# Mariachiar/Spatiotemporal-Deepfake-Detection-for-Live-Video-Calls

Hardware: AMD Instinct MI355X
Metric: clips/sec (32x3x224x224) (higher is better)
Workload: dtype bf16

## Files before the change

### include/af_hip.h

```cpp
#ifndef AF_HIP_H
#define AF_HIP_H

#include <stdint.h>

#ifdef __cplusplus
extern "C" {
#endif

#define AF_ABI_VERSION 6

enum af_dtype { AF_F32 = 0, AF_BF16 = 1, AF_F16 = 2 };

enum af_status {
    AF_OK = 0,
    AF_ERR_ARG = -1,
    AF_ERR_LAUNCH = -2,
    AF_ERR_NO_DEVICE = -3
};

#define AF_STEM_PAD_T 2
#define AF_STEM_PAD_H 3
#define AF_STEM_PAD_W_LEFT 3
#define AF_STEM_PAD_W_TOTAL 8
#define AF_STEM_CPAD 4
// ... 93 lines not shown

int af_conv_cpa_fusable(const af_conv_desc* dc, const af_conv_desc* da, int x_sub);
int af_conv3d_cpa_bn_act(const af_conv_desc* dc, const void* in_b, const void* wc_packed, const float* scale_c, const float* shift_c,
                         const void* residual, void* out_x, int x_sub, const af_conv_desc* da, const void* wa_packed,
                         const float* scale_a, const float* shift_a, void* out_a, void* stream);

int af_conv_variant(const af_conv_desc* d, const af_conv_desc* d2);
const char* af_conv_variant_name(int variant);

int af_maxpool3d(const af_pool_desc* d, const void* in, void* out, void* stream);

int af_avgpool_fc(const af_pool_desc* d, const void* in, const float* fc_w, const float* fc_b,
                  int num_classes, float* pooled, float* logits, void* stream);
int af_avgpool_fc_scores(const af_pool_desc* d, const void* in, const float* fc_w, const float* fc_b,
                         int num_classes, float* pooled, float* logits, float* scores, void* stream);

int af_avgpool(const af_pool_desc* d, const void* in, float* pooled, int pooled_ld, void* stream);
int af_linear(const float* x, const float* w, const float* b, int rows, int in_features, int out_features,
              float* y, void* stream);
int af_linear_scores(const float* x, const float* w, const float* b, int rows, int in_features, int out_features,
                     float* y, float* scores, void* stream);


int af_pack_tstem_weight(const float* w_oidhw, int cout, int kt, int dtype, void* out, void* stream);
long long af_packed_tstem_weight_bytes(int dtype);
int af_tstem_conv_bn_pool_relu(const af_conv_desc* d, const void* stem_in, const void* w_packed, const float* scale,
                               const float* shift, void* out, void* stream);
int af_tstem_conv_bn_pool_relu_maxpool(const af_conv_desc* d, const void* stem_in, const void* w_packed, const float* scale,
                                       const float* shift, void* out, void* stream);

// ... 105 lines not shown
    int64_t in_strides[5];
    float mean[3], std_[3];
    void* workspace;
    int64_t workspace_bytes;
    float* scores;
    const float* scale2;
    const float* shift2;
    af_conv_desc conv3;
    const void* in3;
    const void* weight3;
    const float* scale3;
    const float* shift3;
    af_conv_desc conv4;
    const void* weight4;
    int32_t x_sub;
    int32_t reserved0;
} af_op;

int af_run_ops(const af_op* ops, int n_ops, void* stream);
int af_run_ops_timed(const af_op* ops, int n_ops, void* stream, float* ms);

#define AF_YUNET_MAX_TOPK 8192
#define AF_YUNET_MAX_SIDE 8192
#define AF_YUNET_LAUNCHES 18
typedef struct af_yunet_desc {
    int32_t batch, height, width;
    int32_t top_k;
    int64_t frame_stride, row_pitch;
    float conf_threshold, nms_threshold;
} af_yunet_desc;
int64_t af_yunet_weight_floats(void);
// ... 38 lines not shown
```

### spatiotemporal-deepfake-detection-for-live-video-calls_amd/_lib.py

```python
import ctypes as C
import os

HERE = os.path.dirname(os.path.abspath(__file__))
LIB_PATH = os.environ.get("AF_HIP_LIB") or os.path.join(HERE, "libafhip.so")

AF_F32, AF_BF16, AF_F16 = 0, 1, 2
(AF_OP_STEM, AF_OP_CONV, AF_OP_MAXPOOL, AF_OP_HEAD, AF_OP_PACK_F32, AF_OP_PACK_U8, AF_OP_CONV_DUAL, AF_OP_STEM_POOL, AF_OP_AVGPOOL,
 AF_OP_LINEAR, AF_OP_TSTEM, AF_OP_TOKENS, AF_OP_LAYERNORM, AF_OP_ATTENTION, AF_OP_GELU, AF_OP_CONV_BC, AF_OP_PACK3_F32,
 AF_OP_PACK3_U8, AF_OP_STEM3_POOL, AF_OP_CONV_CA, AF_OP_BLOCK_ABC, AF_OP_TSTEM_POOL3, AF_OP_CONV_CPA) = range(23)
AF_ABI_VERSION = 6
STEM_PAD_T, STEM_PAD_H, STEM_PAD_W_LEFT, STEM_PAD_W_TOTAL, STEM_CPAD = 2, 3, 3, 8, 4

DTYPE_CODES = {"f32": AF_F32, "bf16": AF_BF16, "f16": AF_F16}


class ConvDesc(C.Structure):
    _fields_ = [(n, C.c_int32) for n in (
        "n", "t", "h", "w", "cin", "cout", "kt", "kh", "kw", "st", "sh", "sw", "pt", "ph", "pw",
        "to", "ho", "wo", "relu", "dtype", "tpool")]


class StageRect(C.Structure):
    _fields_ = [("src", C.c_void_p), ("dst_offset", C.c_int64), ("src_pitch", C.c_int64), ("rows", C.c_int32), ("row_bytes", C.c_int32)]

# ... 49 lines not shown
    _fields_ = [
        ("kind", C.c_int32), ("out_ld", C.c_int32),
        ("conv", ConvDesc), ("pool", PoolDesc),
        ("in_", C.c_void_p), ("weight", C.c_void_p), ("scale", C.c_void_p), ("shift", C.c_void_p),
        ("residual", C.c_void_p), ("out", C.c_void_p), ("aux", C.c_void_p),
        ("num_classes", C.c_int32), ("tag", C.c_int32),
        ("conv2", ConvDesc), ("in2", C.c_void_p), ("weight2", C.c_void_p),
        ("in_strides", C.c_int64 * 5),
        ("mean", C.c_float * 3), ("std_", C.c_float * 3),
        ("workspace", C.c_void_p), ("workspace_bytes", C.c_int64),
        ("scores", C.c_void_p),
        ("scale2", C.c_void_p), ("shift2", C.c_void_p),
        ("conv3", ConvDesc), ("in3", C.c_void_p), ("weight3", C.c_void_p),
        ("scale3", C.c_void_p), ("shift3", C.c_void_p),
        ("conv4", ConvDesc), ("weight4", C.c_void_p),
        ("x_sub", C.c_int32), ("reserved0", C.c_int32),
    ]


class YunetDesc(C.Structure):
    _fields_ = [("batch", C.c_int32), ("height", C.c_int32), ("width", C.c_int32), ("top_k", C.c_int32),
                ("frame_stride", C.c_int64), ("row_pitch", C.c_int64), ("conf_threshold", C.c_float), ("nms_threshold", C.c_float)]


YUNET_MAX_TOPK, YUNET_MAX_SIDE, YUNET_LAUNCHES = 8192, 8192, 18


class RetinafaceDesc(C.Structure):
    _fields_ = [("batch", C.c_int32), ("height", C.c_int32), ("width", C.c_int32), ("keep_top_k", C.c_int32),
                ("frame_stride", C.c_int64), ("row_pitch", C.c_int64), ("max_count", C.c_int32), ("reserved", C.c_int32),
                ("min_score", C.c_double)]
# ... 45 lines not shown
    "af_conv_cpa_fusable": (C.c_int, [C.POINTER(ConvDesc)] * 2 + [C.c_int]),
    "af_conv3d_cpa_bn_act": (C.c_int, [C.POINTER(ConvDesc)] + [C.c_void_p] * 6 + [C.c_int, C.POINTER(ConvDesc)] + [C.c_void_p] * 5),
    "af_conv3d_ca_bn_act": (C.c_int, [C.POINTER(ConvDesc), C.c_void_p, C.c_void_p, C.POINTER(ConvDesc)] + [C.c_void_p] * 6
                            + [C.POINTER(ConvDesc)] + [C.c_void_p] * 5),
    "af_conv_bc_fusable": (C.c_int, [C.POINTER(ConvDesc), C.POINTER(ConvDesc)]),
    "af_conv3d_bc_bn_act": (C.c_int, [C.POINTER(ConvDesc)] + [C.c_void_p] * 4 + [C.POINTER(ConvDesc)] + [C.c_void_p] * 5
                            + [C.c_int, C.c_void_p]),
    "af_block_abc_fusable": (C.c_int, [C.POINTER(ConvDesc)] * 4),
    "af_block_abc_bn_act": (C.c_int, ([C.POINTER(ConvDesc)] + [C.c_void_p] * 4) + ([C.POINTER(ConvDesc)] + [C.c_void_p] * 3) * 2
                            + [C.POINTER(ConvDesc), C.c_void_p] + [C.c_void_p, C.c_int, C.c_void_p]),
    "af_conv_variant": (C.c_int, [C.POINTER(ConvDesc), C.POINTER(ConvDesc)]),
    "af_conv_variant_name": (C.c_char_p, [C.c_int]),
    "af_maxpool3d": (C.c_int, [C.POINTER(PoolDesc), C.c_void_p, C.c_void_p, C.c_void_p]),
    "af_avgpool_fc": (C.c_int, [C.POINTER(PoolDesc)] + [C.c_void_p] * 3 + [C.c_int] + [C.c_void_p] * 3),
    "af_avgpool_fc_scores": (C.c_int, [C.POINTER(PoolDesc)] + [C.c_void_p] * 3 + [C.c_int] + [C.c_void_p] * 4),
    "af_linear_scores": (C.c_int, [C.c_void_p] * 3 + [C.c_int] * 3 + [C.c_void_p, C.c_void_p, C.c_void_p]),
    "af_masked_mean_proj": (C.c_int, [C.c_void_p, C.c_int, C.c_int, C.c_int, C.c_void_p, C.c_int, C.c_void_p, C.c_int, C.c_void_p,
                                      C.c_int, C.c_void_p]),
    "af_mlp_head": (C.c_int, [C.c_void_p, C.c_void_p, C.c_int, C.c_int, C.c_int, C.c_void_p, C.c_void_p, C.c_void_p]),
    "af_avgpool": (C.c_int, [C.POINTER(PoolDesc), C.c_void_p, C.c_void_p, C.c_int, C.c_void_p]),
    "af_linear": (C.c_int, [C.c_void_p] * 3 + [C.c_int] * 3 + [C.c_void_p, C.c_void_p]),
    "af_pack_tstem_weight": (C.c_int, [C.c_void_p, C.c_int, C.c_int, C.c_int, C.c_void_p, C.c_void_p]),
    "af_packed_tstem_weight_bytes": (C.c_longlong, [C.c_int]),
    "af_tstem_conv_bn_pool_relu": (C.c_int, [C.POINTER(ConvDesc)] + [C.c_void_p] * 6),
    "af_tstem_conv_bn_pool_relu_maxpool": (C.c_int, [C.POINTER(ConvDesc)] + [C.c_void_p] * 6),
    "af_tokens_assemble": (C.c_int, [C.c_void_p] * 3 + [C.c_int] * 3 + [C.c_void_p, C.c_void_p]),
    "af_layernorm": (C.c_int, [C.c_void_p, C.c_longlong, C.c_void_p, C.c_void_p, C.c_int, C.c_int, C.c_float, C.c_void_p,
                               C.c_longlong, C.c_void_p]),
    "af_attention": (C.c_int, [C.c_void_p, C.c_int, C.c_int, C.c_int, C.c_int, C.c_void_p, C.c_void_p]),
    "af_gelu": (C.c_int, [C.c_void_p, C.c_longlong, C.c_void_p]),
# ... 54 lines not shown
```

### spatiotemporal-deepfake-detection-for-live-video-calls_amd/csrc/af_api.hip

```cpp
#include "af_common.h"

namespace af {

static thread_local char g_err[512] = "";

int set_error(int code, const char* fmt, ...) {
    va_list ap;
    va_start(ap, fmt);
    vsnprintf(g_err, sizeof(g_err), fmt, ap);
    va_end(ap);
    return code;
}

int device_cus() {
    static int cus[kMaxDevices] = {};
    const int dev = current_device();
    if (dev >= 0 && cus[dev] > 0) return cus[dev];
    int n = 0, d = dev < 0 ? 0 : dev;
    if (dev < 0) (void)hipGetDevice(&d);
    if (hipDeviceGetAttribute(&n, hipDeviceAttributeMultiprocessorCount, d) != hipSuccess || n <= 0) n = 256;
    if (dev >= 0) cus[dev] = n;
    return n;
}

static int run_one(const af_op& op, hipStream_t s) {
    switch (op.kind) {
        case AF_OP_STEM:
            return af_stem_conv_bn_relu(&op.conv, op.in, op.weight, op.scale, op.shift, op.out, s);
        case AF_OP_STEM_POOL:
            return af_stem_conv_bn_relu_maxpool(&op.conv, op.in, op.weight, op.scale, op.shift, op.out, s);
        case AF_OP_CONV:
            return af_conv3d_bn_act(&op.conv, op.in, op.weight, op.scale, op.shift, op.residual, op.out, op.out_ld, op.workspace,
                                    op.workspace_bytes, s);
        case AF_OP_CONV_DUAL:
            return af_conv3d_dual_bn_act(&op.conv, op.in, op.weight, &op.conv2, op.in2, op.weight2, op.scale, op.shift,
                                         op.out, op.out_ld, s);
        case AF_OP_CONV_BC:
            return af_conv3d_bc_bn_act(&op.conv, op.in, op.weight, op.scale, op.shift, &op.conv2, op.weight2, op.scale2, op.shift2,
                                       op.residual, op.out, op.out_ld, s);
        case AF_OP_CONV_CPA:
            return af_conv3d_cpa_bn_act(&op.conv, op.in, op.weight, op.scale, op.shift, op.residual, op.out, op.x_sub, &op.conv2,
                                        op.weight2, op.scale2, op.shift2, op.aux, s);
        case AF_OP_CONV_CA:
            return af_conv3d_ca_bn_act(&op.conv, op.in, op.weight, op.in3 ? &op.conv3 : nullptr, op.in3, op.weight3, op.scale, op.shift,
                                       op.residual, op.out, &op.conv2, op.weight2, op.scale2, op.shift2, op.aux, s);
        case AF_OP_BLOCK_ABC:
            return af_block_abc_bn_act(&op.conv, op.in, op.weight, op.scale, op.shift, &op.conv2, op.weight2, op.scale2, op.shift2,
                                       &op.conv3, op.weight3, op.scale3, op.shift3, op.weight4 ? &op.conv4 : nullptr, op.weight4,
                                       op.out, op.out_ld, s);
        case AF_OP_MAXPOOL:
            return af_maxpool3d(&op.pool, op.in, op.out, s);
        case AF_OP_HEAD:
            return af_avgpool_fc_scores(&op.pool, op.in, (const float*)op.weight, op.scale, op.num_classes, (float*)op.aux,
                                        (float*)op.out, op.scores, s);
        case AF_OP_AVGPOOL:
            return af_avgpool(&op.pool, op.in, (float*)op.out, op.out_ld, s);
        case AF_OP_LINEAR:
            return af_linear_scores((const float*)op.in, (const float*)op.weight, op.scale, op.pool.n, op.pool.c, op.num_classes,
                                    (float*)op.out, op.scores, s);
        case AF_OP_PACK_F32:
            return af_pack_input_f32((const float*)op.in, op.conv.n, op.conv.t, op.conv.h, op.conv.w, op.in_strides[0],
                                     op.in_strides[1], op.in_strides[2], op.in_strides[3], op.in_strides[4],
                                     op.conv.dtype, op.out, s);
        case AF_OP_PACK_U8:
            return af_pack_input_u8((const uint8_t*)op.in, op.conv.n, op.conv.t, op.conv.h, op.conv.w, op.mean, op.std_,
                                    op.conv.dtype, op.out, s);
        case AF_OP_STEM3_POOL:
// ... 63 lines not shown
```

### spatiotemporal-deepfake-detection-for-live-video-calls_amd/csrc/af_conv.hip

```cpp
#include "af_common.h"

namespace af {

struct ConvArgs {
    const char* in;
    const char* w;
    const float* scale;
    const float* shift;
    const char* res;
    char* out;
    int T, H, W, Cin, Cout;
    int CinP, CoutP;
    int kt, kh, kw, st, sh, sw, pt, ph, pw;
    int To, Ho, Wo;
    int relu, out_ld;
    int ring;
    int tpool;
    long long M;
    int tiles_n;
    int kpt;
    const char* in2;
    const char* w2;
    int T2, H2, W2, Cin2, Cin2P, st2, sh2, sw2, kpt2;
    int ksplit;
    unsigned div_w_m, div_w_l, div_h_m, div_h_l, div_t_m, div_t_l;
    float* ws;
    long long ws_bytes;
#ifdef AF_STAMPS
    unsigned long long* stamps;
    int dbg;
#endif
};

template <int DT, int BN, int BM, int WN, int WM, int KS, int NSTAGE, int MINW, bool DUAL, bool SPLITK, int BMR>
__device__ __forceinline__ void conv_igemm_tile(const ConvArgs& a, const int bid, const int nb) {
    typedef Elem<DT> E;
    constexpr int EPC = E::EPC;
    constexpr int ES = 16 / EPC;
    constexpr int WTN = BN / WN, WTM = BMR / WM;
    constexpr int TN = WTN / 16, TM = WTM / 16;
    constexpr int NW = WN * WM * KS;
    constexpr int GR = NW * 8;
    constexpr int RW = BN / GR, RX = BM / GR;
    constexpr int PER_WAVE = RW + RX;
    constexpr int STAGE_BYTES = (BN + BM) * 128;
    static_assert(NW == 8 && (KS == 1 || KS == 2) && BN % GR == 0 && BM % GR == 0, "8 waves per workgroup");
    static_assert(BMR <= BM && BMR % (WM * 16) == 0, "real tile rows");
    constexpr bool LEAN = MINW >= 4;
    typedef Mma<DT> MMA;
    static_assert(NSTAGE == 3 || (NSTAGE == 2 && !LEAN && KS == 1), "ring depth of the pipelined loop: 3 or 2 slots");

    extern __shared__ uint4 smem[];
    const unsigned lds0 = (unsigned)(uintptr_t)(__attribute__((address_space(3))) char*)smem;
    AF_STAMP_DECL;
    AF_STAMP(4);

    const int xcd = bid & 7, q = nb >> 3, r = nb & 7;
    const int swz = (xcd < r ? xcd * (q + 1) : r * (q + 1) + (xcd - r) * q) + (bid >> 3);
    const int tile_n = swz % a.tiles_n;
    const int tile_m = swz / a.tiles_n;

    const int tid = threadIdx.x, lane = tid & 63;
// ... 333 lines not shown
        f32x4* red = reinterpret_cast<f32x4*>(smem);
        if (kgroup == 1) {
#pragma unroll
            for (int i = 0; i < TN; ++i)
#pragma unroll
                for (int j = 0; j < TM; ++j) red[(wsub * TN * TM + i * TM + j) * 64 + lane] = acc[i][j];
        }
        __builtin_amdgcn_s_barrier();
        if (kgroup == 1) return;
#pragma unroll
        for (int i = 0; i < TN; ++i)
#pragma unroll
            for (int j = 0; j < TM; ++j) acc[i][j] += red[(wsub * TN * TM + i * TM + j) * 64 + lane];
        patch_off = WN * WM * TN * TM * 64 * 4;
    }
    if constexpr (DT != AF_F32 && !SPLITK && KS == 1 && !LEAN) {
        if (a.tpool == 0 && !a.res) {
            typedef typename E::type OT;
            constexpr int PROW16 = WTN + 8;
            OT* patch16 = reinterpret_cast<OT*>(smem) + wsub * (16 * PROW16);
            constexpr int LPR16 = WTN / 8, RPI16 = 64 / LPR16;
            const int rr16 = lane / LPR16, cc16 = (lane % LPR16) * 8;
            const int chb = tile_n * BN + wn * WTN;
            f32x4 sc[TN], sf[TN];
#pragma unroll
            for (int i = 0; i < TN; ++i) {
                sc[i] = *reinterpret_cast<const f32x4*>(a.scale + chb + i * 16 + fg * 4);
                sf[i] = *reinterpret_cast<const f32x4*>(a.shift + chb + i * 16 + fg * 4);
            }
            const float lo = a.relu ? 0.f : -__builtin_inff();
#pragma unroll
// ... 93 lines not shown
#pragma unroll
                            for (int e = 0; e < EPC; ++e) v[p2][e] += E::to_f32(re[e]);
                        }
                    }
                    uint4 o;
                    typename E::type* oe = reinterpret_cast<typename E::type*>(&o);
#pragma unroll
                    for (int e = 0; e < EPC; ++e) {
                        float x0 = v[0][e], x1 = v[1][e];
                        if (a.relu) { x0 = relu_f(x0); x1 = relu_f(x1); }
                        oe[e] = E::from_f32(max_nan(x0, x1));
                    }
                    __builtin_nontemporal_store(__builtin_bit_cast(u32x4, o), reinterpret_cast<u32x4*>(a.out + ((m >> 1) * a.out_ld + ch0) * ES));
                }
            }
        } else {
#pragma unroll
            for (int it = 0; it < PROWS / RPI; ++it) {
                const int row = it * RPI + rr;
                const long long m = m0 + wm * WTM + hf * PROWS + row;
                float v[EPC];
#pragma unroll
                for (int e = 0; e < EPC; e += 4) {
                    const f32x4 t = *reinterpret_cast<const f32x4*>(patch + row * PROW + cc + e);
                    v[e] = t[0]; v[e + 1] = t[1]; v[e + 2] = t[2]; v[e + 3] = t[3];
                }
                if (SPLITK) {
                    if (m < a.M && ch0 < a.Cout) {
                        float* wp = a.ws + ((long long)blockIdx.y * a.M + m) * a.Cout + ch0;
#pragma unroll
// ... 13 lines not shown
                    }
                    uint4 o;
                    typename E::type* oe = reinterpret_cast<typename E::type*>(&o);
#pragma unroll
                    for (int e = 0; e < EPC; ++e) oe[e] = E::from_f32(v[e]);
                    __builtin_nontemporal_store(__builtin_bit_cast(u32x4, o), reinterpret_cast<u32x4*>(a.out + (m * a.out_ld + ch0) * ES));
                }
            }
        }
        __builtin_amdgcn_wave_barrier();
    }
    AF_STAMP(3); AF_STAMP(7);
    AF_STAMP_FLUSH(bid);
}

template <int DT, int BN, int BM, int WN, int WM, int KS, int NSTAGE, int MINW, bool DUAL, bool SPLITK, int BMR>
__global__ __launch_bounds__(WN * WM * KS * 64, MINW) void conv_igemm_kernel(const ConvArgs a) {
    conv_igemm_tile<DT, BN, BM, WN, WM, KS, NSTAGE, MINW, DUAL, SPLITK, BMR>(a, blockIdx.x, gridDim.x);
}

template <int DT, int BN, int BM, int WN, int WM, int KS, int MINW, bool DUAL, int NSTAGE = 3, bool SPLITK = false, int BMR = BM>
static int launch(const ConvArgs& a, hipStream_t stream) {
    const long long tiles_m = (a.M + BMR - 1) / BMR;
    const long long blocks = tiles_m * a.tiles_n;
    if (blocks <= 0 || blocks > 0x7fffffffLL) return set_error(AF_ERR_ARG, "conv: grid of %lld workgroups", blocks);
    constexpr int TMv = BMR / WM / 16;
    constexpr int red_bytes = KS == 2 ? WN * WM * (BN / WN / 16) * TMv * 64 * 16 : 0;
    constexpr int patch_bytes = red_bytes + WN * WM * ((TMv % 4 == 0 && TMv >= 8 ? TMv / 4 : TMv % 2 == 0 ? TMv / 2 : 1) * 16) * (BN / WN + 4) * 4;
    const int S = a.kt * a.kh * a.kw * a.kpt + a.kpt2;
    const int slots = (MINW >= 4 && a.ring == 2) ? 2 : NSTAGE;
    const int ring_bytes = (S < slots ? S : slots) * (BN + BM) * 128;
    const int lds = ring_bytes > patch_bytes ? ring_bytes : patch_bytes;
    AF_SET_MAX_LDS((&conv_igemm_kernel<DT, BN, BM, WN, WM, KS, NSTAGE, MINW, DUAL, SPLITK, BMR>),
                   NSTAGE * (BN + BM) * 128 > patch_bytes ? NSTAGE * (BN + BM) * 128 : patch_bytes, "conv");
    hipLaunchKernelGGL((conv_igemm_kernel<DT, BN, BM, WN, WM, KS, NSTAGE, MINW, DUAL, SPLITK, BMR>), dim3((unsigned)blocks, SPLITK ? a.ksplit : 1), dim3(WN * WM * KS * 64), lds, stream, a);
    AF_CHECK_LAUNCH("conv_igemm_kernel");
    return AF_OK;
}

enum { VAR_128x256 = 0, VAR_64x256 = 1, VAR_128x128 = 2, VAR_64x128 = 3, VAR_C133 = 4, VAR_128x128_R2 = 5, VAR_256x256 = 6,
       VAR_128x512 = 7, VAR_C311 = 8, VAR_SMALL = 9, VAR_C111 = 10, VAR_C133G = 11, VAR_256x224 = 12, VAR_C311G = 13, VAR_COUNT = 14 };

struct Variant { const char* name; int bn, bm, wn, wm, ks, minw, nstage, bmr, ring; bool dual; };
constexpr Variant variant_info(int v) {
    switch (v) {
        case VAR_128x256: return {"conv_igemm<BN=128,BM=256>", 128, 256, 2, 4, 1, 2, 3, 256, 3, true};
        case VAR_64x256: return {"conv_igemm<BN=64,BM=256>", 64, 256, 1, 8, 1, 2, 3, 256, 3, true};
        case VAR_128x128: return {"conv_igemm<BN=128,BM=128>", 128, 128, 2, 4, 1, 6, 3, 128, 3, true};
        case VAR_128x128_R2: return {"conv_igemm<BN=128,BM=128>", 128, 128, 2, 4, 1, 6, 3, 128, 2, true};
        case VAR_64x128: return {"conv_igemm<BN=64,BM=128>", 64, 128, 1, 8, 1, 4, 3, 128, 3, true};
// ... 91 lines not shown
    constexpr Variant t = variant_info(V < VAR_COUNT ? V : VAR_64x128);
    if constexpr (V < VAR_COUNT && (t.bn == 0 || (DUAL && !t.dual))) return launch_variant<DT, DUAL, SPLITK, V + 1>(v, a, stream);
    else {
        if constexpr (V < VAR_COUNT) if (v != V) return launch_variant<DT, DUAL, SPLITK, V + 1>(v, a, stream);
        return launch<DT, t.bn, t.bm, t.wn, t.wm, t.ks, t.minw, DUAL, t.nstage, SPLITK, t.bmr>(a, stream);
    }
}

template <int DT>
static int dispatch(ConvArgs& a, const ConvPad& p, int v, hipStream_t stream) {
    a.kpt = p.kpt; a.CinP = p.cinp; a.kpt2 = p.kpt2; a.Cin2P = p.cin2p; a.CoutP = p.coutp;
    a.tiles_n = a.CoutP / variant_bn(v);
    a.ring = variant_info(v).ring;
    a.ksplit = plan_ksplit(v, a.M, a.CoutP, a.Cout, p.ksteps, a.tpool, a.in2 != nullptr);
    if (a.ksplit > 1 && (!a.ws || a.ws_bytes < (long long)a.ksplit * a.M * a.Cout * (long long)sizeof(float))) a.ksplit = 1;
    const int rc = a.in2 ? launch_variant<DT, true, false>(v, a, stream)
                   : a.ksplit > 1 ? launch_variant<DT, false, true>(v, a, stream) : launch_variant<DT, false, false>(v, a, stream);
    if (rc != AF_OK || a.ksplit == 1) return rc;
    const long long quads = a.M * (a.Cout / 4);
    hipLaunchKernelGGL((splitk_finish_kernel<DT>), dim3((unsigned)((quads + 255) / 256)), dim3(256), 0, stream, a.ws, a.ksplit, a.M, a.Cout,
                       a.scale, a.shift, a.res, a.relu, a.out, a.out_ld);
    AF_CHECK_LAUNCH("splitk_finish_kernel");
    return AF_OK;
}

}

extern "C" int af_conv_variant(const af_conv_desc* d, const af_conv_desc* d2) {
    AF_REQUIRE(d && d->cout > 0 && d->cin > 0 && af::dtype_ok(d->dtype), "conv_variant: bad descriptor");
    return af::conv_path(d, d2, nullptr, 0, af::conv_pad(d, d2));
}

extern "C" const char* af_conv_variant_name(int variant) {
    return af::variant_info(variant).name;
}

extern "C" int64_t af_conv_workspace_bytes(const af_conv_desc* d) {
    using namespace af;
    if (!d || d->cout <= 0 || d->cin <= 0 || !dtype_ok(d->dtype) || d->n <= 0 || d->to <= 0 || d->ho <= 0 || d->wo <= 0) return 0;
    const ConvPad p = conv_pad(d, nullptr);
    const int ks = plan_ksplit(pick_variant(d, p), p.M, p.coutp, d->cout, p.ksteps, d->tpool, false);
    return ks > 1 ? (int64_t)ks * p.M * d->cout * (int64_t)sizeof(float) : 0;
}

static int conv_common(const af_conv_desc* d, const void* in, const void* w_packed, const af_conv_desc* d2,
                       const void* in2, const void* w2_packed, const float* scale, const float* shift,
                       const void* residual, void* out, int out_ld, void* workspace, int64_t workspace_bytes, void* stream) {
    using namespace af;
    AF_REQUIRE(d && in && w_packed && scale && shift && out, "conv: null argument");
    AF_REQUIRE(dtype_ok(d->dtype), "conv: bad dtype %d", d->dtype);
    AF_REQUIRE(d->n > 0 && d->t > 0 && d->h > 0 && d->w > 0 && d->cin > 0 && d->cout > 0, "conv: bad dims");
    AF_REQUIRE(d->kt > 0 && d->kh > 0 && d->kw > 0 && d->st > 0 && d->sh > 0 && d->sw > 0, "conv: bad kernel/stride");
    AF_REQUIRE(d->pt >= 0 && d->ph >= 0 && d->pw >= 0, "conv: negative padding");
    const int to = (d->t + 2 * d->pt - d->kt) / d->st + 1, ho = (d->h + 2 * d->ph - d->kh) / d->sh + 1,
              wo = (d->w + 2 * d->pw - d->kw) / d->sw + 1;
    AF_REQUIRE(to == d->to && ho == d->ho && wo == d->wo && to > 0 && ho > 0 && wo > 0,
               "conv: output dims (%d,%d,%d) do not match the descriptor (%d,%d,%d)", to, ho, wo, d->to, d->ho, d->wo);
    const int bk = d->dtype == AF_F32 ? 32 : 64, epc = d->dtype == AF_F32 ? 4 : 8;
    AF_REQUIRE(d->cin % epc == 0, "conv: cin=%d must be a multiple of %d for this dtype", d->cin, epc);
    AF_REQUIRE(d->cout % epc == 0, "conv: cout=%d must be a multiple of %d for this dtype", d->cout, epc);
    if (out_ld == 0) out_ld = d->cout;
    AF_REQUIRE(out_ld >= d->cout && out_ld % 8 == 0, "conv: bad out_ld %d", out_ld);
    AF_REQUIRE(aligned16(in) && aligned16(w_packed) && aligned16(scale) && aligned16(shift) && aligned16(out) &&
                   aligned16(residual), "conv: buffers must be 16-byte aligned");
    AF_REQUIRE((long long)(d->cout + 63) * d->kt * d->kh * d->kw * (d->cin + bk) < (1LL << 31), "conv: weight too large");
    AF_REQUIRE(d->kt * d->kh * d->kw <= 31, "conv: at most 31 kernel taps (got %d)", d->kt * d->kh * d->kw);
    AF_REQUIRE((long long)d->kt * d->h * d->w * d->cin * dtype_size(d->dtype) < (1LL << 31), "conv: tap offset overflows");
    AF_REQUIRE(2 * d->pt <= d->kt && 2 * d->ph <= d->kh && 2 * d->pw <= d->kw, "conv: padding larger than half the kernel");
    AF_REQUIRE((256 / ((long long)to * ho * wo) + 3) * d->t * d->h * d->w * d->cin * dtype_size(d->dtype) < (1LL << 31),
               "conv: one clip of input is too large for 32-bit tile offsets");

    const ConvPad p = conv_pad(d, d2);
    const int path = conv_path(d, d2, residual, out_ld, p);
    switch (path) {
        case VAR_C133: return conv133_run(d, in, w_packed, scale, shift, out, (hipStream_t)stream);
        case VAR_C133G: return conv133g_run(d, in, w_packed, scale, shift, out, out_ld, (hipStream_t)stream);
        case VAR_C311G: return conv311g_run(d, in, w_packed, scale, shift, out, out_ld, (hipStream_t)stream);
        case VAR_C311: return conv311_run(d, in, w_packed, scale, shift, out, out_ld, (hipStream_t)stream);
        default: break;
    }
    ConvArgs a;
    a.in = (const char*)in; a.w = (const char*)w_packed; a.scale = scale; a.shift = shift;
    a.res = (const char*)residual; a.out = (char*)out;
    a.T = d->t; a.H = d->h; a.W = d->w; a.Cin = d->cin; a.Cout = d->cout;
    a.kt = d->kt; a.kh = d->kh; a.kw = d->kw; a.st = d->st; a.sh = d->sh; a.sw = d->sw;
    a.pt = d->pt; a.ph = d->ph; a.pw = d->pw; a.To = to; a.Ho = ho; a.Wo = wo;
    a.relu = d->relu; a.out_ld = out_ld;
    AF_REQUIRE(aligned16(workspace) && workspace_bytes >= 0, "conv: the workspace must be 16-byte aligned");
    a.ws = (float*)workspace; a.ws_bytes = workspace ? workspace_bytes : 0;
    fill_stamps(a, "AF_G_DBG");
    AF_REQUIRE(d->tpool >= 0 && d->tpool <= 2, "conv: tpool must be 0, 1 (temporal pairs) or 2 (2x2 pixels)");
    a.tpool = d->tpool;
    AF_REQUIRE(a.tpool != 1 || (to % 2 == 0), "conv: fused temporal pool needs an even number of output frames (%d)", to);
    AF_REQUIRE(a.tpool != 2 || (ho % 2 == 0 && wo % 2 == 0 && !residual && !d2),
               "conv: the fused 2x2 pool needs even output height / width (%d x %d), no residual and no second segment", ho, wo);
    a.M = (long long)d->n * to * ho * wo;
    AF_REQUIRE(a.M < (1LL << 31), "conv: %lld output positions (the row index is 32-bit)", a.M);
    {
        auto magic = [](unsigned dv, unsigned& mm, unsigned& l) {
            l = 0; while ((1ull << l) < dv) ++l;
            mm = (unsigned)(((1ull << 32) * ((1ull << l) - dv)) / dv + 1);
        };
        magic((unsigned)(a.tpool == 2 ? (wo >> 1) : wo), a.div_w_m, a.div_w_l);
        magic((unsigned)(a.tpool == 2 ? (ho >> 1) : ho), a.div_h_m, a.div_h_l);
// ... 14 lines not shown
        a.T2 = d2->t; a.H2 = d2->h; a.W2 = d2->w; a.Cin2 = d2->cin; a.st2 = d2->st; a.sh2 = d2->sh; a.sw2 = d2->sw;
    }
    if (path == VAR_SMALL)
        return conv_small_run(d, in, w_packed, d2, in2, w2_packed, scale, shift, residual, out, out_ld, (hipStream_t)stream);
    if (path == VAR_C111)
        return conv111_run(d, in, w_packed, d2, in2, w2_packed, scale, shift, residual, out, out_ld, (hipStream_t)stream);
    return with_dtype(d->dtype, [&](auto dt) { return dispatch<dt>(a, p, path, (hipStream_t)stream); });
}

extern "C" int af_conv3d_bn_act(const af_conv_desc* d, const void* in, const void* w_packed, const float* scale,
                                const float* shift, const void* residual, void* out, int out_ld, void* workspace,
                                int64_t workspace_bytes, void* stream) {
    return conv_common(d, in, w_packed, nullptr, nullptr, nullptr, scale, shift, residual, out, out_ld, workspace, workspace_bytes, stream);
}

extern "C" int af_conv_ca_fusable(const af_conv_desc* dc, const af_conv_desc* d1, const af_conv_desc* da) {
    return af::conv_ca_applies(dc, d1, da) ? 1 : 0;
}

extern "C" int af_conv3d_ca_bn_act(const af_conv_desc* dc, const void* in_b, const void* wc_packed, const af_conv_desc* d1,
                                   const void* in1, const void* w1_packed, const float* scale_c, const float* shift_c,
                                   const void* residual, void* out_x, const af_conv_desc* da, const void* wa_packed,
                                   const float* scale_a, const float* shift_a, void* out_a, void* stream) {
    using namespace af;
    AF_REQUIRE(dc && da && in_b && wc_packed && scale_c && shift_c && out_x && wa_packed && scale_a && shift_a && out_a, "conv_ca: null argument");
    AF_REQUIRE((d1 != nullptr) == (in1 != nullptr) && (d1 != nullptr) == (w1_packed != nullptr) && (d1 != nullptr) != (residual != nullptr),
               "conv_ca: either a residual (plain block) or the projection shortcut (d1, in1, w1: block 0), not both");
    AF_REQUIRE(aligned16(in_b) && aligned16(wc_packed) && aligned16(in1) && aligned16(w1_packed) && aligned16(scale_c) && aligned16(shift_c) &&
                   aligned16(residual) && aligned16(out_x) && aligned16(wa_packed) && aligned16(scale_a) && aligned16(shift_a) && aligned16(out_a),
               "conv_ca: buffers must be 16-byte aligned");
// ... 33 lines not shown
```

### spatiotemporal-deepfake-detection-for-live-video-calls_amd/csrc/af_pool.hip

```cpp
#include "af_common.h"

namespace af {

struct PoolArgs {
    const char* in; char* out;
    int T, H, W, C;
    int kt, kh, kw, st, sh, sw, pt, ph, pw;
    int To, Ho, Wo;
    int out_ld;
    long long total;
};

template <int DT>
__global__ void maxpool_kernel(const PoolArgs a) {
    typedef typename Elem<DT>::type elem_t;
    constexpr int V = Elem<DT>::EPC;
    long long idx = (long long)blockIdx.x * blockDim.x + threadIdx.x;
    if (idx >= a.total) return;
    const int cg = a.C / V;
    int c = (int)(idx % cg) * V; long long r = idx / cg;
    int wo = (int)(r % a.Wo); r /= a.Wo;
    int ho = (int)(r % a.Ho); r /= a.Ho;
    int to = (int)(r % a.To); long long n = r / a.To;
    float best[V];
// ... 69 lines not shown

__global__ void fc_kernel(const float* __restrict__ pooled, const float* __restrict__ w, const float* __restrict__ b,
                          int C, int num_classes, float* __restrict__ logits, float* __restrict__ scores) {
    __shared__ float red[4];
    const long long row = blockIdx.x;
    float l0 = 0.f, l1 = 0.f;
    for (int k = 0; k < num_classes; ++k) {
        float s = 0.f;
        for (int c = threadIdx.x; c < C; c += blockDim.x) s += pooled[row * C + c] * w[(long long)k * C + c];
#pragma unroll
        for (int o = 32; o > 0; o >>= 1) s += __shfl_down(s, o, 64);
        if ((threadIdx.x & 63) == 0) red[threadIdx.x >> 6] = s;
        __syncthreads();
        if (threadIdx.x == 0) {
            const float l = red[0] + red[1] + red[2] + red[3] + b[k];
            logits[row * num_classes + k] = l;
            if (k == 0) l0 = l; else if (k == 1) l1 = l;
        }
        __syncthreads();
    }
    if (scores && threadIdx.x == 0)
        scores[row] = num_classes == 1 ? 1.f / (1.f + expf(-l0)) : 1.f / (1.f + expf(l0 - l1));
}

}

using namespace af;

static int check_pool(const af_pool_desc* d, const char* what, bool need_vec) {
    AF_REQUIRE(d && dtype_ok(d->dtype), "%s: bad descriptor", what);
// ... 86 lines not shown
                                    int num_classes, float* pooled, float* logits, float* scores, void* stream) {
    AF_REQUIRE(in && fc_w && fc_b && pooled && logits && num_classes > 0, "avgpool_fc: null argument");
    AF_REQUIRE(!scores || num_classes == 1 || num_classes == 2,
               "avgpool_fc: scores are defined for 1 (sigmoid) or 2 (softmax[:,1]) classes, got %d", num_classes);
    int rc = check_avgpool(d, "avgpool_fc");
    if (rc) return rc;
    rc = launch_avgpool(d, in, pooled, d->c, (hipStream_t)stream);
    if (rc) return rc;
    return af_linear_scores(pooled, fc_w, fc_b, d->n * d->to * d->ho * d->wo, d->c, num_classes, logits, scores, stream);
}

extern "C" int af_avgpool_fc(const af_pool_desc* d, const void* in, const float* fc_w, const float* fc_b,
                             int num_classes, float* pooled, float* logits, void* stream) {
    return af_avgpool_fc_scores(d, in, fc_w, fc_b, num_classes, pooled, logits, nullptr, stream);
}
```

### spatiotemporal-deepfake-detection-for-live-video-calls_amd/engine.py

```python
import ctypes as C
import dataclasses
import os
from typing import Dict, List, Optional

import torch

from . import _lib
from ._lib import Op, check, lib
from .arch import BN_EPS, ConvSpec, FtcnTTSpec, NetSpec, PoolSpec, SlowFastSpec

_TORCH_DTYPE = {"f32": torch.float32, "bf16": torch.bfloat16, "f16": torch.float16}
_ELEM_SIZE = {"f32": 4, "bf16": 2, "f16": 2}

TAG_PACK, TAG_STEM, TAG_POOL, TAG_HEAD = 0, 1, 2, 3
TAG_CONV_1x1x1, TAG_CONV_Tx1x1, TAG_CONV_1x3x3, TAG_CONV_OTHER, TAG_CONV_BC, TAG_CONV_CA, TAG_BLOCK_ABC = 10, 11, 12, 13, 14, 15, 16
TAG_NAMES = {TAG_PACK: "input_pack", TAG_STEM: "stem", TAG_POOL: "maxpool", TAG_HEAD: "head",
             TAG_CONV_1x1x1: "conv_1x1x1", TAG_CONV_Tx1x1: "conv_3x1x1", TAG_CONV_1x3x3: "conv_1x3x3",
             TAG_CONV_OTHER: "conv_other", TAG_CONV_BC: "conv_1x3x3+1x1x1_fused", TAG_CONV_CA: "conv_1x1x1+3x1x1_fused",
             TAG_BLOCK_ABC: "bottleneck_block_fused"}


def _conv_tag(cv: ConvSpec) -> int:
    k = tuple(cv.kernel)
    if k == (1, 1, 1):
# ... 445 lines not shown
            if e["kind"] == "tt_head":
                self._materialise_tt_head(n_pack + k, e)
                continue
            name, macs = self._EMIT[e["kind"]](self, op, e)
            self.op_names.append(name)
            self.op_macs.append(batch * macs)
        need = 0
        for i in range(self.n_ops):
            if self.ops[i].kind == _lib.AF_OP_CONV:
                need = max(need, int(lib.af_conv_workspace_bytes(C.byref(self.ops[i].conv))))
        self.workspace = torch.empty(need // 4, dtype=torch.float32, device=device) if need else None
        for i in range(self.n_ops):
            if self.ops[i].kind == _lib.AF_OP_CONV and need:
                self.ops[i].workspace = self.workspace.data_ptr()
                self.ops[i].workspace_bytes = need

    def _at(self, buf: Optional[str]):
        return self.buf[buf].data_ptr() if buf else None

    def _desc(self, cv: ConvSpec, din, dout, relu=True, tpool=0):
        return _conv_desc(self.batch, self.code, cv, din, dout, relu, tpool)

    def _pool_desc(self, e, kernel, stride=(1, 1, 1), pad=(0, 0, 0)):
        return _lib.pool_desc(self.batch, e["din"], e["ch"], kernel, stride, pad, self.code, e["dout"], e.get("ld", 0))

    _CONV_KINDS = {"stem": _lib.AF_OP_STEM, "stem_pool": _lib.AF_OP_STEM_POOL, "stem3_pool": _lib.AF_OP_STEM3_POOL,
                   "tstem": _lib.AF_OP_TSTEM, "tstem_pool3": _lib.AF_OP_TSTEM_POOL3, "conv": _lib.AF_OP_CONV}

    def _emit_conv(self, op, e):
        cv: ConvSpec = e["cv"]
# ... 217 lines not shown
        assert clips.dtype == torch.uint8 and clips.is_cuda
        if len(self.inputs) != 1:
            raise ValueError("the uint8 prologue is wired for single-input networks")
        B, T, H, W, Cc = clips.shape
        if (B, T, H, W, Cc) != (self.batch,) + self.in_dims + (3,) or not clips.is_contiguous():
            raise ValueError("expected contiguous uint8 clips (%d,%d,%d,%d,3)" % ((self.batch,) + self.in_dims))
        pk = self.ops[0]
        pk.kind = self.k_pack_u8
        pk.in_ = clips.data_ptr()
        for i in range(3):
            pk.mean[i], pk.std_[i] = float(mean[i]), float(std[i])
        check(lib.af_run_ops(self.ops, self.n_ops, _stream_ptr(self.device)), "af_run_ops")
        return self.logits, self.pooled

    def run_prefix(self, n_ops: int):
        check(lib.af_run_ops(self.ops, n_ops, _stream_ptr(self.device)), "af_run_ops")

    def run_timed(self, first_op: int = 0):
        ms = (C.c_float * self.n_ops)()
        n = self.n_ops - first_op
        ops = C.cast(C.addressof(self.ops) + first_op * C.sizeof(Op), C.POINTER(Op))
        msp = C.cast(C.addressof(ms) + first_op * C.sizeof(C.c_float), C.POINTER(C.c_float))
        check(lib.af_run_ops_timed(ops, n, _stream_ptr(self.device), msp), "af_run_ops_timed")
        return [float(v) for v in ms]

    def activation(self, op_index: int) -> torch.Tensor:
        op = self.ops[op_index]
        if op.kind in (_lib.AF_OP_STEM_POOL, _lib.AF_OP_STEM3_POOL, _lib.AF_OP_TSTEM_POOL3):
            shape = (op.conv.n, op.conv.to, (op.conv.ho - 1) // 2 + 1, (op.conv.wo - 1) // 2 + 1, op.conv.cout)
        elif op.kind == _lib.AF_OP_CONV_BC:
            shape = (op.conv2.n, op.conv2.to, op.conv2.ho, op.conv2.wo, op.out_ld or op.conv2.cout)
# ... 19 lines not shown
```

Measured before the change: 3459.

## Fuse final residual conv epilogue with global average pool for the head

The last residual conv before the classifier head now reduces its activated output into per-16-row group sums directly in the epilogue, instead of writing the full activation tensor. A new head kernel sums those group partials per clip, divides by the position count, and runs the FC and score computation. This removes the write and re-read of the final feature map and the separate pooling pass. In exchange it forces ksplit=1 on that layer and adds a two-slot scheme for groups that straddle clip boundaries. run_prefix disables the fusion so intermediate activations stay available.

```diff
diff --git a/include/af_hip.h b/include/af_hip.h
--- a/include/af_hip.h
+++ b/include/af_hip.h
@@ -131,6 +131,13 @@
                   int num_classes, float* pooled, float* logits, void* stream);
 int af_avgpool_fc_scores(const af_pool_desc* d, const void* in, const float* fc_w, const float* fc_b,
                          int num_classes, float* pooled, float* logits, float* scores, void* stream);
+
+int af_conv_headpool_fusable(const af_conv_desc* d, const af_pool_desc* pool);
+int64_t af_conv_headpool_bytes(const af_conv_desc* d);
+int af_conv3d_bn_act_headpool(const af_conv_desc* d, const af_pool_desc* pool, const void* in, const void* w_packed,
+                              const float* scale, const float* shift, const void* residual, float* group_sums, void* stream);
+int af_headpool_fc_scores(const float* group_sums, int n, int rows_per_clip, int c, const float* fc_w, const float* fc_b,
+                          int num_classes, float* pooled, float* logits, float* scores, void* stream);
 
 int af_avgpool(const af_pool_desc* d, const void* in, float* pooled, int pooled_ld, void* stream);
 int af_linear(const float* x, const float* w, const float* b, int rows, int in_features, int out_features,
@@ -266,7 +273,7 @@
     af_conv_desc conv4;
     const void* weight4;
     int32_t x_sub;
-    int32_t reserved0;
+    int32_t head_fuse;
 } af_op;
 
 int af_run_ops(const af_op* ops, int n_ops, void* stream);
diff --git a/spatiotemporal-deepfake-detection-for-live-video-calls_amd/_lib.py b/spatiotemporal-deepfake-detection-for-live-video-calls_amd/_lib.py
--- a/spatiotemporal-deepfake-detection-for-live-video-calls_amd/_lib.py
+++ b/spatiotemporal-deepfake-detection-for-live-video-calls_amd/_lib.py
@@ -87,7 +87,7 @@
         ("conv3", ConvDesc), ("in3", C.c_void_p), ("weight3", C.c_void_p),
         ("scale3", C.c_void_p), ("shift3", C.c_void_p),
         ("conv4", ConvDesc), ("weight4", C.c_void_p),
-        ("x_sub", C.c_int32), ("reserved0", C.c_int32),
+        ("x_sub", C.c_int32), ("head_fuse", C.c_int32),
     ]
 
 
@@ -163,6 +163,10 @@
     "af_maxpool3d": (C.c_int, [C.POINTER(PoolDesc), C.c_void_p, C.c_void_p, C.c_void_p]),
     "af_avgpool_fc": (C.c_int, [C.POINTER(PoolDesc)] + [C.c_void_p] * 3 + [C.c_int] + [C.c_void_p] * 3),
     "af_avgpool_fc_scores": (C.c_int, [C.POINTER(PoolDesc)] + [C.c_void_p] * 3 + [C.c_int] + [C.c_void_p] * 4),
+    "af_conv_headpool_fusable": (C.c_int, [C.POINTER(ConvDesc), C.POINTER(PoolDesc)]),
+    "af_conv_headpool_bytes": (C.c_int64, [C.POINTER(ConvDesc)]),
+    "af_conv3d_bn_act_headpool": (C.c_int, [C.POINTER(ConvDesc), C.POINTER(PoolDesc)] + [C.c_void_p] * 7),
+    "af_headpool_fc_scores": (C.c_int, [C.c_void_p] + [C.c_int] * 3 + [C.c_void_p] * 2 + [C.c_int] + [C.c_void_p] * 4),
     "af_linear_scores": (C.c_int, [C.c_void_p] * 3 + [C.c_int] * 3 + [C.c_void_p, C.c_void_p, C.c_void_p]),
     "af_masked_mean_proj": (C.c_int, [C.c_void_p, C.c_int, C.c_int, C.c_int, C.c_void_p, C.c_int, C.c_void_p, C.c_int, C.c_void_p,
                                       C.c_int, C.c_void_p]),
diff --git a/spatiotemporal-deepfake-detection-for-live-video-calls_amd/csrc/af_api.hip b/spatiotemporal-deepfake-detection-for-live-video-calls_amd/csrc/af_api.hip
--- a/spatiotemporal-deepfake-detection-for-live-video-calls_amd/csrc/af_api.hip
+++ b/spatiotemporal-deepfake-detection-for-live-video-calls_amd/csrc/af_api.hip
@@ -30,6 +30,8 @@
         case AF_OP_STEM_POOL:
             return af_stem_conv_bn_relu_maxpool(&op.conv, op.in, op.weight, op.scale, op.shift, op.out, s);
         case AF_OP_CONV:
+            if (op.head_fuse)
+                return af_conv3d_bn_act_headpool(&op.conv, &op.pool, op.in, op.weight, op.scale, op.shift, op.residual, (float*)op.aux, s);
             return af_conv3d_bn_act(&op.conv, op.in, op.weight, op.scale, op.shift, op.residual, op.out, op.out_ld, op.workspace,
                                     op.workspace_bytes, s);
         case AF_OP_CONV_DUAL:
@@ -51,6 +53,10 @@
         case AF_OP_MAXPOOL:
             return af_maxpool3d(&op.pool, op.in, op.out, s);
         case AF_OP_HEAD:
+            if (op.head_fuse)
+                return af_headpool_fc_scores((const float*)op.in2, op.pool.n, op.pool.kt * op.pool.kh * op.pool.kw, op.pool.c,
+                                             (const float*)op.weight, op.scale, op.num_classes, (float*)op.aux, (float*)op.out,
+                                             op.scores, s);
             return af_avgpool_fc_scores(&op.pool, op.in, (const float*)op.weight, op.scale, op.num_classes, (float*)op.aux,
                                         (float*)op.out, op.scores, s);
         case AF_OP_AVGPOOL:
diff --git a/spatiotemporal-deepfake-detection-for-live-video-calls_amd/csrc/af_conv.hip b/spatiotemporal-deepfake-detection-for-live-video-calls_amd/csrc/af_conv.hip
--- a/spatiotemporal-deepfake-detection-for-live-video-calls_amd/csrc/af_conv.hip
+++ b/spatiotemporal-deepfake-detection-for-live-video-calls_amd/csrc/af_conv.hip
@@ -26,13 +26,15 @@
     unsigned div_w_m, div_w_l, div_h_m, div_h_l, div_t_m, div_t_l;
     float* ws;
     long long ws_bytes;
+    float* pool;
+    int pool_rows, pool_slots;
 #ifdef AF_STAMPS
     unsigned long long* stamps;
     int dbg;
 #endif
 };
 
-template <int DT, int BN, int BM, int WN, int WM, int KS, int NSTAGE, int MINW, bool DUAL, bool SPLITK, int BMR>
+template <int DT, int BN, int BM, int WN, int WM, int KS, int NSTAGE, int MINW, bool DUAL, bool SPLITK, int BMR, bool POOL>
 __device__ __forceinline__ void conv_igemm_tile(const ConvArgs& a, const int bid, const int nb) {
     typedef Elem<DT> E;
     constexpr int EPC = E::EPC;
@@ -46,6 +48,7 @@
     constexpr int STAGE_BYTES = (BN + BM) * 128;
     static_assert(NW == 8 && (KS == 1 || KS == 2) && BN % GR == 0 && BM % GR == 0, "8 waves per workgroup");
     static_assert(BMR <= BM && BMR % (WM * 16) == 0, "real tile rows");
+    static_assert(!POOL || (!SPLITK && !DUAL && KS == 1), "the pooled epilogue: one input, whole K, every wave in the epilogue");
     constexpr bool LEAN = MINW >= 4;
     typedef Mma<DT> MMA;
     static_assert(NSTAGE == 3 || (NSTAGE == 2 && !LEAN && KS == 1), "ring depth of the pipelined loop: 3 or 2 slots");
@@ -409,7 +412,7 @@
             for (int j = 0; j < TM; ++j) acc[i][j] += red[(wsub * TN * TM + i * TM + j) * 64 + lane];
         patch_off = WN * WM * TN * TM * 64 * 4;
     }
-    if constexpr (DT != AF_F32 && !SPLITK && KS == 1 && !LEAN) {
+    if constexpr (DT != AF_F32 && !SPLITK && KS == 1 && !LEAN && !POOL) {
         if (a.tpool == 0 && !a.res) {
             typedef typename E::type OT;
             constexpr int PROW16 = WTN + 8;
@@ -533,6 +536,51 @@
                     __builtin_nontemporal_store(__builtin_bit_cast(u32x4, o), reinterpret_cast<u32x4*>(a.out + ((m >> 1) * a.out_ld + ch0) * ES));
                 }
             }
+        } else if constexpr (POOL) {
+            constexpr int IPG = 16 / RPI;
+            static_assert(RPI <= 16 && 16 % RPI == 0 && PROWS % 16 == 0, "row groups of the pooled epilogue");
+#pragma unroll
+            for (int g = 0; g < PROWS / 16; ++g) {
+                const unsigned mg = (unsigned)m0 + wm * WTM + hf * PROWS + g * 16;
+                const unsigned mb = a.pool_slots == 2 ? (mg / (unsigned)a.pool_rows + 1) * (unsigned)a.pool_rows : 0xffffffffu;
+                const int passes = (mb < mg + 16 && mb < (unsigned)a.M) ? 2 : 1;
+                for (int sl = 0; sl < passes; ++sl) {
+                    float gs[EPC];
+#pragma unroll
+                    for (int e = 0; e < EPC; ++e) gs[e] = 0.f;
+#pragma unroll
+                    for (int i2 = 0; i2 < IPG; ++i2) {
+                        const int row = g * 16 + i2 * RPI + rr;
+                        const unsigned m = mg + i2 * RPI + rr;
+                        if (m < (unsigned)a.M && ch0 < a.Cout && (m >= mb) == (sl == 1)) {
+                            float v[EPC];
+#pragma unroll
+                            for (int e = 0; e < EPC; e += 4) {
+                                const f32x4 t = *reinterpret_cast<const f32x4*>(patch + row * PROW + cc + e);
+                                v[e] = t[0]; v[e + 1] = t[1]; v[e + 2] = t[2]; v[e + 3] = t[3];
+                            }
+                            if (a.res) {
+                                const uint4 rraw = __builtin_bit_cast(uint4, __builtin_nontemporal_load(reinterpret_cast<const u32x4*>(a.res + ((long long)m * a.Cout + ch0) * ES)));
+                                const typename E::type* re = reinterpret_cast<const typename E::type*>(&rraw);
+#pragma unroll
+                                for (int e = 0; e < EPC; ++e) v[e] += E::to_f32(re[e]);
+                            }
+#pragma unroll
+                            for (int e = 0; e < EPC; ++e) gs[e] += E::to_f32(E::from_f32(a.relu ? relu_f(v[e]) : v[e]));
+                        }
+                    }
+#pragma unroll
+                    for (int o = LPR; o < 64; o <<= 1)
+#pragma unroll
+                        for (int e = 0; e < EPC; ++e) gs[e] += __shfl_xor(gs[e], o, 64);
+                    if (rr == 0 && mg < (unsigned)a.M && ch0 < a.Cout) {
+                        float* gp = a.pool + ((long long)(mg >> 4) * a.pool_slots + sl) * a.Cout + ch0;
+#pragma unroll
+                        for (int e = 0; e < EPC; e += 4)
+                            *reinterpret_cast<f32x4*>(gp + e) = f32x4{gs[e], gs[e + 1], gs[e + 2], gs[e + 3]};
+                    }
+                }
+            }
         } else {
 #pragma unroll
             for (int it = 0; it < PROWS / RPI; ++it) {
@@ -576,12 +624,12 @@
     AF_STAMP_FLUSH(bid);
 }
 
-template <int DT, int BN, int BM, int WN, int WM, int KS, int NSTAGE, int MINW, bool DUAL, bool SPLITK, int BMR>
+template <int DT, int BN, int BM, int WN, int WM, int KS, int NSTAGE, int MINW, bool DUAL, bool SPLITK, int BMR, bool POOL = false>
 __global__ __launch_bounds__(WN * WM * KS * 64, MINW) void conv_igemm_kernel(const ConvArgs a) {
-    conv_igemm_tile<DT, BN, BM, WN, WM, KS, NSTAGE, MINW, DUAL, SPLITK, BMR>(a, blockIdx.x, gridDim.x);
-}
-
-template <int DT, int BN, int BM, int WN, int WM, int KS, int MINW, bool DUAL, int NSTAGE = 3, bool SPLITK = false, int BMR = BM>
+    conv_igemm_tile<DT, BN, BM, WN, WM, KS, NSTAGE, MINW, DUAL, SPLITK, BMR, POOL>(a, blockIdx.x, gridDim.x);
+}
+
+template <int DT, int BN, int BM, int WN, int WM, int KS, int MINW, bool DUAL, int NSTAGE = 3, bool SPLITK = false, int BMR = BM, bool POOL = false>
 static int launch(const ConvArgs& a, hipStream_t stream) {
     const long long tiles_m = (a.M + BMR - 1) / BMR;
     const long long blocks = tiles_m * a.tiles_n;
@@ -593,9 +641,9 @@
     const int slots = (MINW >= 4 && a.ring == 2) ? 2 : NSTAGE;
     const int ring_bytes = (S < slots ? S : slots) * (BN + BM) * 128;
     const int lds = ring_bytes > patch_bytes ? ring_bytes : patch_bytes;
-    AF_SET_MAX_LDS((&conv_igemm_kernel<DT, BN, BM, WN, WM, KS, NSTAGE, MINW, DUAL, SPLITK, BMR>),
+    AF_SET_MAX_LDS((&conv_igemm_kernel<DT, BN, BM, WN, WM, KS, NSTAGE, MINW, DUAL, SPLITK, BMR, POOL>),
                    NSTAGE * (BN + BM) * 128 > patch_bytes ? NSTAGE * (BN + BM) * 128 : patch_bytes, "conv");
-    hipLaunchKernelGGL((conv_igemm_kernel<DT, BN, BM, WN, WM, KS, NSTAGE, MINW, DUAL, SPLITK, BMR>), dim3((unsigned)blocks, SPLITK ? a.ksplit : 1), dim3(WN * WM * KS * 64), lds, stream, a);
+    hipLaunchKernelGGL((conv_igemm_kernel<DT, BN, BM, WN, WM, KS, NSTAGE, MINW, DUAL, SPLITK, BMR, POOL>), dim3((unsigned)blocks, SPLITK ? a.ksplit : 1), dim3(WN * WM * KS * 64), lds, stream, a);
     AF_CHECK_LAUNCH("conv_igemm_kernel");
     return AF_OK;
 }
@@ -717,6 +765,12 @@
     a.ring = variant_info(v).ring;
     a.ksplit = plan_ksplit(v, a.M, a.CoutP, a.Cout, p.ksteps, a.tpool, a.in2 != nullptr);
     if (a.ksplit > 1 && (!a.ws || a.ws_bytes < (long long)a.ksplit * a.M * a.Cout * (long long)sizeof(float))) a.ksplit = 1;
+    if (a.pool) {
+        a.ksplit = 1;
+        constexpr Variant t = variant_info(VAR_128x128), u = variant_info(VAR_64x128);
+        if (v == VAR_64x128) return launch<DT, u.bn, u.bm, u.wn, u.wm, u.ks, u.minw, false, u.nstage, false, u.bmr, true>(a, stream);
+        return launch<DT, t.bn, t.bm, t.wn, t.wm, t.ks, t.minw, false, t.nstage, false, t.bmr, true>(a, stream);
+    }
     const int rc = a.in2 ? launch_variant<DT, true, false>(v, a, stream)
                    : a.ksplit > 1 ? launch_variant<DT, false, true>(v, a, stream) : launch_variant<DT, false, false>(v, a, stream);
     if (rc != AF_OK || a.ksplit == 1) return rc;
@@ -746,9 +800,24 @@
     return ks > 1 ? (int64_t)ks * p.M * d->cout * (int64_t)sizeof(float) : 0;
 }
 
+static bool conv_headpool_applies(const af_conv_desc* d, const af_pool_desc* pl) {
+    using namespace af;
+    if (!d || !pl || !dtype_ok(d->dtype) || d->cout <= 0 || d->cin <= 0 || d->n <= 0 || d->to <= 0 || d->ho <= 0 || d->wo <= 0) return false;
+    if (d->tpool || pl->dtype != d->dtype || pl->n != d->n || pl->c != d->cout) return false;
+    if (pl->t != d->to || pl->h != d->ho || pl->w != d->wo || pl->kt != d->to || pl->kh != d->ho || pl->kw != d->wo) return false;
+    if (pl->to != 1 || pl->ho != 1 || pl->wo != 1 || pl->st != 1 || pl->sh != 1 || pl->sw != 1 || pl->pt || pl->ph || pl->pw) return false;
+    const long long rows = (long long)d->to * d->ho * d->wo;
+    if (rows < 16 || d->cout % (d->dtype == AF_F32 ? 4 : 8) != 0) return false;
+    const ConvPad p = conv_pad(d, nullptr);
+    const int v = conv_path(d, nullptr,  d, d->cout, p);
+    if (v != VAR_128x128 && v != VAR_128x128_R2 && v != VAR_64x128) return false;
+    return plan_ksplit(v, p.M, p.coutp, d->cout, p.ksteps, 0, false) == 1;
+}
+
 static int conv_common(const af_conv_desc* d, const void* in, const void* w_packed, const af_conv_desc* d2,
                        const void* in2, const void* w2_packed, const float* scale, const float* shift,
-                       const void* residual, void* out, int out_ld, void* workspace, int64_t workspace_bytes, void* stream) {
+                       const void* residual, void* out, int out_ld, void* workspace, int64_t workspace_bytes, void* stream,
+                       float* pool = nullptr) {
     using namespace af;
     AF_REQUIRE(d && in && w_packed && scale && shift && out, "conv: null argument");
     AF_REQUIRE(dtype_ok(d->dtype), "conv: bad dtype %d", d->dtype);
@@ -775,6 +844,7 @@
 
     const ConvPad p = conv_pad(d, d2);
     const int path = conv_path(d, d2, residual, out_ld, p);
+    AF_REQUIRE(!pool || path == VAR_128x128 || path == VAR_128x128_R2 || path == VAR_64x128, "conv_headpool: this layer does not run on a 128-row lean tile");
     switch (path) {
         case VAR_C133: return conv133_run(d, in, w_packed, scale, shift, out, (hipStream_t)stream);
         case VAR_C133G: return conv133g_run(d, in, w_packed, scale, shift, out, out_ld, (hipStream_t)stream);
@@ -791,6 +861,7 @@
     a.relu = d->relu; a.out_ld = out_ld;
     AF_REQUIRE(aligned16(workspace) && workspace_bytes >= 0, "conv: the workspace must be 16-byte aligned");
     a.ws = (float*)workspace; a.ws_bytes = workspace ? workspace_bytes : 0;
+    a.pool = pool; a.pool_rows = to * ho * wo; a.pool_slots = a.pool_rows % 16 ? 2 : 1;
     fill_stamps(a, "AF_G_DBG");
     AF_REQUIRE(d->tpool >= 0 && d->tpool <= 2, "conv: tpool must be 0, 1 (temporal pairs) or 2 (2x2 pixels)");
     a.tpool = d->tpool;
@@ -835,6 +906,24 @@
     return conv_common(d, in, w_packed, nullptr, nullptr, nullptr, scale, shift, residual, out, out_ld, workspace, workspace_bytes, stream);
 }
 
+extern "C" int af_conv_headpool_fusable(const af_conv_desc* d, const af_pool_desc* pool) {
+    return conv_headpool_applies(d, pool) ? 1 : 0;
+}
+
+extern "C" int64_t af_conv_headpool_bytes(const af_conv_desc* d) {
+    if (!d || d->n <= 0 || d->to <= 0 || d->ho <= 0 || d->wo <= 0 || d->cout <= 0) return 0;
+    const int64_t rows = (int64_t)d->to * d->ho * d->wo;
+    return (d->n * rows + 15) / 16 * (rows % 16 ? 2 : 1) * d->cout * (int64_t)sizeof(float);
+}
+
+extern "C" int af_conv3d_bn_act_headpool(const af_conv_desc* d, const af_pool_desc* pool, const void* in, const void* w_packed,
+                                         const float* scale, const float* shift, const void* residual, float* group_sums,
+                                         void* stream) {
+    AF_REQUIRE(d && pool && group_sums && af::aligned16(group_sums), "conv_headpool: null or unaligned argument");
+    AF_REQUIRE(conv_headpool_applies(d, pool), "conv_headpool: this (conv, pool) pair does not take the fused path (ask af_conv_headpool_fusable first)");
+    return conv_common(d, in, w_packed, nullptr, nullptr, nullptr, scale, shift, residual, group_sums, d->cout, nullptr, 0, stream, group_sums);
+}
+
 extern "C" int af_conv_ca_fusable(const af_conv_desc* dc, const af_conv_desc* d1, const af_conv_desc* da) {
     return af::conv_ca_applies(dc, d1, da) ? 1 : 0;
 }
diff --git a/spatiotemporal-deepfake-detection-for-live-video-calls_amd/csrc/af_pool.hip b/spatiotemporal-deepfake-detection-for-live-video-calls_amd/csrc/af_pool.hip
--- a/spatiotemporal-deepfake-detection-for-live-video-calls_amd/csrc/af_pool.hip
+++ b/spatiotemporal-deepfake-detection-for-live-video-calls_amd/csrc/af_pool.hip
@@ -107,6 +107,44 @@
         __syncthreads();
         if (threadIdx.x == 0) {
             const float l = red[0] + red[1] + red[2] + red[3] + b[k];
+            logits[row * num_classes + k] = l;
+            if (k == 0) l0 = l; else if (k == 1) l1 = l;
+        }
+        __syncthreads();
+    }
+    if (scores && threadIdx.x == 0)
+        scores[row] = num_classes == 1 ? 1.f / (1.f + expf(-l0)) : 1.f / (1.f + expf(l0 - l1));
+}
+
+__global__ __launch_bounds__(1024) void headpool_fc_kernel(const float* __restrict__ sums, int rows, int slots, const float* __restrict__ w,
+                                                           const float* __restrict__ b, int C, int num_classes, float* __restrict__ pooled,
+                                                           float* __restrict__ logits, float* __restrict__ scores) {
+    __shared__ float red[16];
+    const long long row = blockIdx.x;
+    const long long r0 = row * rows;
+    const int g0 = (int)(r0 >> 4), groups = (int)((r0 + rows - 1) >> 4) - g0 + 1;
+    const float* sp = sums + (long long)g0 * slots * C;
+    const int first = (r0 & 15) ? C : 0;
+    for (int c = threadIdx.x * 4; c < C; c += blockDim.x * 4) {
+        f32x4 t = f32x4{0.f, 0.f, 0.f, 0.f};
+#pragma unroll 7
+        for (int g = 0; g < groups; ++g) t += *reinterpret_cast<const f32x4*>(sp + (long long)g * slots * C + (g == 0 ? first : 0) + c);
+        *reinterpret_cast<f32x4*>(pooled + row * C + c) = t / (float)rows;
+    }
+    __syncthreads();
+    const int nw = blockDim.x >> 6;
+    float l0 = 0.f, l1 = 0.f;
+    for (int k = 0; k < num_classes; ++k) {
+        float s = 0.f;
+        for (int c = threadIdx.x; c < C; c += blockDim.x) s += pooled[row * C + c] * w[(long long)k * C + c];
+#pragma unroll
+        for (int o = 32; o > 0; o >>= 1) s += __shfl_down(s, o, 64);
+        if ((threadIdx.x & 63) == 0) red[threadIdx.x >> 6] = s;
+        __syncthreads();
+        if (threadIdx.x == 0) {
+            float l = 0.f;
+            for (int i = 0; i < nw; ++i) l += red[i];
+            l += b[k];
             logits[row * num_classes + k] = l;
             if (k == 0) l0 = l; else if (k == 1) l1 = l;
         }
@@ -223,3 +261,16 @@
                              int num_classes, float* pooled, float* logits, void* stream) {
     return af_avgpool_fc_scores(d, in, fc_w, fc_b, num_classes, pooled, logits, nullptr, stream);
 }
+
+extern "C" int af_headpool_fc_scores(const float* group_sums, int n, int rows_per_clip, int c, const float* fc_w, const float* fc_b,
+                                     int num_classes, float* pooled, float* logits, float* scores, void* stream) {
+    AF_REQUIRE(group_sums && fc_w && fc_b && pooled && logits && n > 0 && c > 0 && num_classes > 0, "headpool_fc: bad argument");
+    AF_REQUIRE(rows_per_clip >= 16, "headpool_fc: a clip has %d positions, fewer than a 16-row group", rows_per_clip);
+    AF_REQUIRE(c % 4 == 0 && aligned16(group_sums) && aligned16(pooled), "headpool_fc: 16-byte rows (c = %d)", c);
+    AF_REQUIRE(!scores || num_classes == 1 || num_classes == 2, "headpool_fc: scores are defined for 1 (sigmoid) or 2 (softmax[:,1]) classes, got %d",
+               num_classes);
+    hipLaunchKernelGGL(headpool_fc_kernel, dim3((unsigned)n), dim3(c >= 4096 ? 1024 : c >= 1024 ? 512 : 256), 0, (hipStream_t)stream, group_sums,
+                       rows_per_clip, rows_per_clip % 16 ? 2 : 1, fc_w, fc_b, c, num_classes, pooled, logits, scores);
+    AF_CHECK_LAUNCH("headpool_fc_kernel");
+    return AF_OK;
+}
diff --git a/spatiotemporal-deepfake-detection-for-live-video-calls_amd/engine.py b/spatiotemporal-deepfake-detection-for-live-video-calls_amd/engine.py
--- a/spatiotemporal-deepfake-detection-for-live-video-calls_amd/engine.py
+++ b/spatiotemporal-deepfake-detection-for-live-video-calls_amd/engine.py
@@ -483,6 +483,20 @@
             if self.ops[i].kind == _lib.AF_OP_CONV and need:
                 self.ops[i].workspace = self.workspace.data_ptr()
                 self.ops[i].workspace_bytes = need
+        self.head_fused, self.head_sums = None, None
+        for i in range(1, self.n_ops):
+            cv, hd = self.ops[i - 1], self.ops[i]
+            if (hd.kind == _lib.AF_OP_HEAD and cv.kind == _lib.AF_OP_CONV and cv.residual and cv.out == hd.in_
+                    and cv.out_ld in (0, cv.conv.cout) and lib.af_conv_headpool_fusable(C.byref(cv.conv), C.byref(hd.pool))):
+                self.head_sums = torch.empty(int(lib.af_conv_headpool_bytes(C.byref(cv.conv))) // 4, dtype=torch.float32, device=device)
+                cv.pool = hd.pool
+                cv.aux = hd.in2 = self.head_sums.data_ptr()
+                self.head_fused = (i - 1, i)
+        self._set_head_fuse(1)
+
+    def _set_head_fuse(self, on: int):
+        for i in self.head_fused or ():
+            self.ops[i].head_fuse = on
 
     def _at(self, buf: Optional[str]):
         return self.buf[buf].data_ptr() if buf else None
@@ -730,7 +744,11 @@
         return self.logits, self.pooled
 
     def run_prefix(self, n_ops: int):
-        check(lib.af_run_ops(self.ops, n_ops, _stream_ptr(self.device)), "af_run_ops")
+        self._set_head_fuse(0)
+        try:
+            check(lib.af_run_ops(self.ops, n_ops, _stream_ptr(self.device)), "af_run_ops")
+        finally:
+            self._set_head_fuse(1)
 
     def run_timed(self, first_op: int = 0):
         ms = (C.c_float * self.n_ops)()
```

Result: no change. 3448 (-0.3%).
